# draessld/EDSParser

Measured on AMD Instinct MI355X. Metric: msa2eds_input_MB_per_s, higher is better.
Workload: dtype u8

## Files before the change

### edsparser_amd/csrc/msa_fast_kernels.hpp

```cpp
#pragma once
#include "msa_generic_kernels.hpp"

namespace edsx {

constexpr u64 META_REC = 1ull << 63;
constexpr u64 META_KIND4 = 1ull << 62;
constexpr u64 META_INLINE = 1ull << 61;
constexpr u64 META_KIND8 = 1ull << 60;
constexpr u64 META_RECID = (1ull << 40) - 1;
constexpr u64 CNT_SCATTER = 1ull << 63;
constexpr u64 CNT_SLOT = (1ull << 48) - 1;
constexpr u64 CNT_MIXED = 1ull << 62;
constexpr u32 REC_H_SLOT = 8, REC_H_REP = 16;

__global__ void __launch_bounds__(256) k_seg_meta(FastParams p)
{
    const MsaView& mv = p.mv;
    if (mv.hdr->status) return;
    const u64 nseg = *p.nseg_ptr;
    const u64 p0 = mv.vbit(0) ? 0 : 1;
    const u64 nvs = nseg > p0 ? (nseg - p0 + 1) / 2 : 0;
    if (blockIdx.x == 0 && threadIdx.x == 0) mv.hdr->nvs = nvs;
    auto common = [&](u64 seg, u64 a, u64 b) {
        p.eds_len[seg] = 2 + (b - a);
// ... 11 lines not shown
        if (vi == 0 && p0) common(0, p.seg_start[0], a);
        if (seg + 1 < nseg) common(seg + 1, b, p.seg_start[seg + 2]);
        u64 work_cm = 0, work_wide = 0, work_wide16 = 0;
        bool done = false;
        if (p.Fraw && ((p.Fraw[a >> 6] >> (a & 63)) & 1ull)) {
            const u64 slot = mv.slot(a);
            const u32 info = p.rec_info[slot];
            if (info >> 31) {
                p.eds_len[seg] = (info >> 8) & 0xffu;
                p.seds_len[seg] = (u64)(info & 0xffu) + p.tok_total;
                p.segmeta[seg] = META_REC | META_INLINE | ((info >> 30) & 1u ? META_KIND4 : 0) | slot;
                work_wide = ((info >> 30) & 1u) && (info & 0xffu) <= 8u;
                work_wide16 = ((info >> 30) & 1u) && (info & 0xffu) > 8u;
                done = true;
            }
        }
        if (!done) {
            u64 cm = 0;
            const u64 ncol = b - a;
            if (ncol <= 64) {
                const u64 s0 = mv.slot(a);
                bool pure = true, contig = true;
                for (u64 c = a + 1; c < b; c++) {
                    pure = pure && mv.vbit(c);
                    if (pure) contig = contig && mv.slot(c) == s0 + (c - a);
                }
                if (pure) cm = (ncol << 48) | s0 | (contig ? 0 : CNT_SCATTER);
                else cm = (ncol << 48) | s0 | CNT_MIXED;
            }
            if (!cm) p.slow_list[atomicAdd(p.slow_count, 1ull)] = seg;
            p.segmeta[seg] = 0;
            work_cm = cm;
        }
        const bool heavy = work_cm && ((work_cm & CNT_MIXED) || ((work_cm >> 48) & 0xffu) > 10u);
        p.cnt_meta[vi] = work_cm; p.cnt_flag[vi] = work_cm && !heavy ? 1 : 0; p.heavy_flag[vi] = heavy ? 1 : 0;
        p.wide_flag[vi] = work_wide; p.wide16_flag[vi] = work_wide16;
    }
}

__global__ void __launch_bounds__(256) k_work_scatter(FastParams p, const u64* __restrict__ pos, const u64* __restrict__ hpos,
                                                      const u64* __restrict__ nvs_ptr)
{
    if (p.mv.hdr->status) return;
    const u64 nvs = *nvs_ptr;
    for (u64 vi = blockIdx.x * (u64)blockDim.x + threadIdx.x; vi < nvs; vi += (u64)gridDim.x * blockDim.x) {
        const u64 cm = p.cnt_meta[vi];
        if (cm) {
            const bool heavy = (cm & CNT_MIXED) || ((cm >> 48) & 0xffu) > 10u;
            if (heavy) { const u64 i = hpos[vi]; p.heavy_vi[i] = vi; p.heavy_cm[i] = cm; }
            else { const u64 i = pos[vi]; p.cnt_vi[i] = vi; p.cnt_cm[i] = cm; }
        }
        const u64 wpos = p.wide_flag[vi];
        const u64 wnext = vi + 1 < nvs ? p.wide_flag[vi + 1] : *p.wide_count;
        if (wnext != wpos) p.wide_list[wpos] = vi;
        const u64 xpos = p.wide16_flag[vi];
        const u64 xnext = vi + 1 < nvs ? p.wide16_flag[vi + 1] : *p.wide16_count;
        if (xnext != xpos) p.wide16_list[xpos] = vi;
    }
}

__device__ __forceinline__ uint32_t lut32(const u32* t, uint32_t g4)
{
    const uint32_t sel = g4 & 0x07070707u;
    const uint32_t h3 = (g4 >> 3) & 0x01010101u, m3 = (h3 << 8) - h3;
    const uint32_t h4 = (g4 >> 4) & 0x01010101u, m4 = (h4 << 8) - h4;
    const uint32_t e0 = __builtin_amdgcn_perm(t[1], t[0], sel), e1 = __builtin_amdgcn_perm(t[3], t[2], sel);
    const uint32_t e2 = __builtin_amdgcn_perm(t[5], t[4], sel), e3 = __builtin_amdgcn_perm(t[7], t[6], sel);
    const uint32_t lo = (e1 & m3) | (e0 & ~m3), hi = (e3 & m3) | (e2 & ~m3);
    return (hi & m4) | (lo & ~m4);
}

__device__ __forceinline__ uint32_t lut64(const u32* t, uint32_t g4)
{
    const uint32_t h5 = (g4 >> 5) & 0x01010101u, m5 = (h5 << 8) - h5;
    return (lut32(t + 8, g4) & m5) | (lut32(t, g4) & ~m5);
}

template <int MAXG> __device__ __forceinline__ uint32_t lutN(const u32* t, uint32_t g4)
{
    if constexpr (MAXG <= 8) return __builtin_amdgcn_perm(t[1], t[0], g4);
    else if constexpr (MAXG <= 16) {
// ... 125 lines not shown
    if (ncol == 1) {
        if (fast_group_dna1(col0, rb, vmask, lane, mv.S, G)) return 1;
        G.gid = make_uint4(~0u, ~0u, ~0u, ~0u);
        G.k = 0; G.sumlen = 0; G.key_lo = 0; G.key_hi = 0; G.rep = 0; G.len = 0;
        if (ballot64(any_nul(col0, vmask))) return 0;
        const uint4 col = normalise_col<CHECK_NL>(col0, vmask, saw_nl);
        while (first_remaining(rm, leader, i0)) {
            const u32 c = leader_byte(col, leader, i0);
            uint4 eq = bytes_eq_mask(col, c * 0x01010101u);
            eq.x &= rm.x; eq.y &= rm.y; eq.z &= rm.z; eq.w &= rm.w;
            if (!fast_assign(G, rm, eq, (u64)c, 0ull, c ? 1u : 0u, lane, (u32)leader * 16u + i0)) return 0;
        }
        return 1;
    }

    const u64 slot0 = cmeta & CNT_SLOT;
    const bool scatter = (cmeta & CNT_SCATTER) != 0, mixed = (cmeta & CNT_MIXED) != 0;
    if (mixed && !HEAVY) return 2;
    const u32 loff = lane * 16u < mv.Spad - 16u ? lane * 16u : mv.Spad - 16u;
    const uint8_t* cbase = mv.vc + slot0 * (u64)mv.Spad + loff;
    u32 nA = ncol;
    const uint8_t* cbaseB = cbase;
    const bool two = scatter && mv.lw == 0 && mv.tileW != 0;
    if (two) {
        const u64 bnd = (seg_a / mv.tileW + 1) * mv.tileW;
        nA = (u32)(bnd - seg_a);
        cbaseB = mv.vc + uniform64(mv.word_slot[bnd >> 6]) * (u64)mv.Spad + loff;
    }
    auto col_ptr = [&](u32 c) -> const uint8_t* {
        if (two) return c < nA ? cbase + (u64)c * mv.Spad : cbaseB + (u64)(c - nA) * mv.Spad;
        return scatter ? mv.vc + mv.slot(seg_a + c) * (u64)mv.Spad + loff : cbase + (u64)c * mv.Spad;
    };

    if (!HEAVY && ncol > 10u) return 2;
    if (ncol <= 10u && !mixed) {
        auto load_col = [&](u32 c) -> uint4 { return load16u(col_ptr(c)); };
        const int r = fast_group_dnakeys<1>(load_col, ncol, col0, lane, vmask, G);
        if (r) return r > 0 ? 1 : 0;
        G.gid = make_uint4(~0u, ~0u, ~0u, ~0u);
        G.k = 0; G.sumlen = 0; G.key_lo = 0; G.key_hi = 0; G.rep = 0; G.len = 0;
    }
    if constexpr (HEAVY) {
        if (ncol > 10u && ncol <= 20u && !mixed) {
            auto load_col = [&](u32 c) -> uint4 { return load16u(col_ptr(c)); };
            const int r = fast_group_dnakeys<2>(load_col, ncol, col0, lane, vmask, G);
            if (r) return r > 0 ? 1 : 0;
            G.gid = make_uint4(~0u, ~0u, ~0u, ~0u);
            G.k = 0; G.sumlen = 0; G.key_lo = 0; G.key_hi = 0; G.rep = 0; G.len = 0;
        }
        auto cell_ptr = [&](u32 c) -> const uint8_t* {
            const uint8_t* cp = two ? (c < nA ? cbase + (u64)c * mv.Spad : cbaseB + (u64)(c - nA) * mv.Spad)
                                    : (scatter ? mv.vc + mv.slot(seg_a + c) * (u64)mv.Spad + loff : cbase + (u64)c * mv.Spad);
            return cp - loff;
        };
        u32 cs_lo = 0, cs_hi = 0, cref = 0x100u;
        if (mixed && lane < ncol) {
            if (mv.vbit(seg_a + lane)) { const u64 sl = mv.slot(seg_a + lane); cs_lo = (u32)sl; cs_hi = (u32)(sl >> 32); }
            else cref = mv.ref_byte(seg_a + lane);
        }
        auto load_colx = [&](u32 c) -> uint4 {
            if (mixed) {
                const u32 rb = (u32)__builtin_amdgcn_readlane((int)cref, (int)c);
                if (rb < 0x100u) { const u32 b = rb * 0x01010101u; return make_uint4(b, b, b, b); }
                const u64 sl = ((u64)(u32)__builtin_amdgcn_readlane((int)cs_hi, (int)c) << 32) | (u32)__builtin_amdgcn_readlane((int)cs_lo, (int)c);
                return load16u(mv.vc + sl * (u64)mv.Spad + loff);
            }
            return load16u(col_ptr(c));
        };
        auto cell = [&](u32 c, u32 row) -> u32 {
            if (row == ~0u) return mixed ? (u32)__builtin_amdgcn_readlane((int)cref, (int)c) : 0x100u;
            if (mixed) return cref < 0x100u ? cref : (u32)mv.vc[(((u64)cs_hi << 32) | cs_lo) * (u64)mv.Spad + row];
            return (u32)cell_ptr(c)[row];
        };
        if (mv.S <= 64u && !mixed) {
            const bool act = lane < mv.S;
            u32* const mine32 = reinterpret_cast<u32*>(strs + lane * 64u);
// ... 712 lines not shown
```

### edsparser_amd/csrc/msa_scan_kernels.hpp

```cpp
#pragma once
#include "msa_wave.hpp"
#include "msa_scan_launch.hpp"

namespace edsx {

__global__ void k_find_hdr_end(const uint8_t* __restrict__ f, u64 n, MsaHdr* h)
{
    const u32 lane = threadIdx.x;
    h->first_nl = n;
    h->first_hdr2 = n;
    if (n == 0 || f[0] != '>') {
        if (lane == 0) { h->status |= ST_NOT_FASTA; h->hdr_end = n; }
        return;
    }
    u64 pos = n;
    for (u64 base = 0; base < n; base += 64) {
        u64 i = base + lane;
        u64 b = ballot64(i < n && f[i] == '\n');
        if (b) { pos = base + __builtin_ctzll(b); break; }
    }
    if (lane == 0) h->hdr_end = pos;
}

__global__ void __launch_bounds__(1024) k_find_row0(const uint8_t* __restrict__ f, u64 n, MsaHdr* h)
// ... 147 lines not shown
            u64 nonnl = 0;
            for (u64 i = lane; i < rest; i += 64) nonnl |= (f[p + i] != '\n');
            if (ballot64(nonnl != 0)) bad = ST_LAYOUT;
            break;
        }
        u64 nlpos = n;
        u64 b = ballot64(lane >= 2 && c == '\n');
        if (b) nlpos = q + __builtin_ctzll(b);
        else {
            for (u64 base = q + 64; base < n; base += 64) {
                const u64 i = base + lane;
                b = ballot64(i < n && f[i] == '\n');
                if (b) { nlpos = base + __builtin_ctzll(b); break; }
            }
        }
        if (nlpos >= n) { bad = ST_LAYOUT; break; }
        st = nlpos + 1;
    }
    if (lane == 0) {
        if (s < 2 && !bad) bad = ST_FEW_ROWS;
        h->status |= bad;
        h->S = s; h->L = L; h->lw = wrapped ? lw : 0; h->Draw = Draw;
        h->nwords = (L + 63) / 64;
        h->nwords_raw = (Draw + 63) / 64;
    }
}

__global__ void k_pad_rows(u64* __restrict__ row_start, u64 S, u64 n)
{
    const u64 last = row_start[S - 1];
    for (u64 r = S + blockIdx.x * (u64)blockDim.x + threadIdx.x; r < n; r += (u64)gridDim.x * blockDim.x) row_start[r] = last;
}

constexpr u32 FUSE_MAXW = 10;
#ifndef EDSX_TAIL_WAVES
#define EDSX_TAIL_WAVES 8
#endif
constexpr u32 TAIL_WAVES = EDSX_TAIL_WAVES;
constexpr u32 CLIST = 2048;



template <bool ROWS64>
__device__ __forceinline__ void fused_group_run(const K1Params& p, const uint8_t* colbuf, u32 desc, u64 slot_base, u32 lane,
                                                const uint4& vmask, u32 nl, u32 loff)
{
    const u32 idx0 = desc & 0x7ffu, w = desc >> 11;
    const uint8_t* c0p = colbuf + (size_t)idx0 * p.Spad;
    FastGroups G;
    G.gid = make_uint4(~0u, ~0u, ~0u, ~0u);
    G.k = 0; G.sumlen = 0; G.key_lo = 0; G.key_hi = 0; G.rep = 0; G.len = 0;
    bool ok;
    if constexpr (ROWS64) {
        const bool act = lane < p.S;
        const u64 LET = ((u64)DNA_LET_HI << 32) | DNA_LET_LO;
        u32 klo = 0, khi = 0, len = 0, bad = 0;
        for (u32 c = 0; c < w; c++) {
            const u32 ch = act ? (u32)c0p[(size_t)c * p.Spad + lane] : (u32)'-';
            const u32 cls = ((ch >> 1) ^ (ch >> 2)) & 7u;
            bad |= ((u32)(LET >> (8u * cls)) & 0xffu) != ch ? 1u : 0u;
            if (cls != 5u) { if (len < 10u) klo |= cls << (3u * len); else khi |= cls << (3u * (len - 10u)); len++; }
        }
        ok = !ballot64(act && bad);
        u32 mygid = 0, gk_lo = 0, gk_hi = 0, glen = 0;
        if (ok) {
            u64 todo = ballot64(act);
            while (todo) {
// ... 95 lines not shown
    const u64 q = q0 + (u64)j * 16;
    const bool full_tile = q0 + (u64)cpr * 16 <= p.Draw;
    const int nb = q < p.Draw ? ((p.Draw - q) < 16 ? (int)(p.Draw - q) : 16) : 0;
    const u32 valid = nb == 16 ? 0xffffu : ((1u << nb) - 1u);

    constexpr bool DIRECT_OK = HOLD && LANEROWS;
    const bool direct = DIRECT_OK && full_tile;
    const u64* rs = BIG ? p.row_start : reinterpret_cast<const u64*>(colbuf);
    if (!direct && !BIG) for (u32 r = tid; r < p.S; r += T) reinterpret_cast<u64*>(colbuf)[r] = p.row_start[r];
    if (tid < 256) { D[tid] = 0; CS[tid] = 0; }
    if (tid == 0) { ncand_sh = 0; nst_sh = 0; }
    if (!direct) __syncthreads();

    const uint8_t* f = p.file;
    const u32 Sm1 = p.S - 1;
    auto row_of = [&](u32 it) -> u32 {
        if constexpr (LANEROWS) return sub * 16u + it;
        else return sub + it * RI;
    };
    uint4 ref = make_uint4(0, 0, 0, 0);
    uint4 d[HOLD ? RPT : 1];
    uint4 acc = make_uint4(0, 0, 0, 0);
    if (direct) {
        if constexpr (DIRECT_OK) {
            ref = load16u(f + p.row_start[0] + q);
            const ulonglong2* rp = reinterpret_cast<const ulonglong2*>(p.row_start + sub * 16u);
            ulonglong2 rv[8];
#pragma unroll
            for (int i = 0; i < 8; i++) rv[i] = rp[i];
#pragma unroll
            for (int i = 0; i < 8; i++) { d[2 * i] = load16u(f + rv[i].x + q); d[2 * i + 1] = load16u(f + rv[i].y + q); }
#pragma unroll
            for (int it = 0; it < RPT; it++) {
                acc.x |= d[it].x ^ ref.x; acc.y |= d[it].y ^ ref.y;
                acc.z |= d[it].z ^ ref.z; acc.w |= d[it].w ^ ref.w;
            }
        }
    } else if (full_tile) {
        ref = load16u(f + rs[0] + q);
#pragma unroll
        for (int it = 0; it < RPT; it++) {
            const u32 r = row_of(it);
            d[HOLD ? it : 0] = load16u(f + rs[r < p.S ? r : Sm1] + q);
            if constexpr (!HOLD) {
                acc.x |= d[0].x ^ ref.x; acc.y |= d[0].y ^ ref.y; acc.z |= d[0].z ^ ref.z; acc.w |= d[0].w ^ ref.w;
            }
        }
        if constexpr (HOLD) {
#pragma unroll
            for (int it = 0; it < RPT; it++) {
                acc.x |= d[it].x ^ ref.x; acc.y |= d[it].y ^ ref.y;
                acc.z |= d[it].z ^ ref.z; acc.w |= d[it].w ^ ref.w;
            }
        }
    } else {
        if (nb > 0) ref = load_partial(f + rs[0] + q, nb);
#pragma unroll
        for (int it = 0; it < RPT; it++) {
            const u32 r = row_of(it);
            uint4 v = ref;
            if (r < p.S && nb > 0) v = load_partial(f + rs[r] + q, nb);
            d[HOLD ? it : 0] = v;
            acc.x |= v.x ^ ref.x; acc.y |= v.y ^ ref.y; acc.z |= v.z ^ ref.z; acc.w |= v.w ^ ref.w;
        }
    }
    if constexpr (!HOLD) {
        for (u32 r = sub + RPT * RI; r < p.S; r += RI) {
            if (nb > 0) {
                const uint8_t* src = f + rs[r] + q;
                uint4 v = nb == 16 ? load16u(src) : load_partial(src, nb);
                acc.x |= v.x ^ ref.x; acc.y |= v.y ^ ref.y; acc.z |= v.z ^ ref.z; acc.w |= v.w ^ ref.w;
            }
        }
    }
    u32 diff = chunk_ne16(acc, make_uint4(0, 0, 0, 0));
    diff |= chunk_eq16(ref, 0x2d2d2d2du);
    diff &= valid;
    u32 bad = 0;
    u32 nlmask = 0;
    if (p.lw && nb > 0) {
        u64 m = q % (p.lw + 1);
        for (int i = 0; i < nb; i++) { if (m == p.lw) { nlmask |= 1u << i; m = 0; } else m++; }
    }
    if ((chunk_eq16(ref, 0x0a0a0a0au) & valid) != nlmask) bad = 1;
    if (direct) {
        for (u32 o = cpr; o < 64u; o <<= 1) diff |= (u32)__shfl_xor((int)diff, (int)o, 64);
        __syncthreads();
        if ((tid & 63u) < cpr && diff) atomicOr(&D[j], diff);
    } else if (diff) atomicOr(&D[j], diff);
    __syncthreads();

    const u32 V16 = D[j];
    if (V16 & nlmask) bad = 1;

    const bool fastpre = cpr <= 8u;
    u64 prepk = 0;
    u32 w0 = 0, w1 = 0, w2 = 0, w3 = 0, nv = 0;
    if (fastpre) {
        const uint4 da = *reinterpret_cast<const uint4*>(&D[0]), db = *reinterpret_cast<const uint4*>(&D[4]);
        const u32 dm[8] = {uniform32(da.x), uniform32(da.y), uniform32(da.z), uniform32(da.w),
                           uniform32(db.x), uniform32(db.y), uniform32(db.z), uniform32(db.w)};
#pragma unroll
        for (int c = 0; c < 8; c++) { prepk |= (u64)nv << (8 * c); nv += (u32)__builtin_popcount(dm[c]); }
    } else {
        if (tid < 256) {
            u32 c = tid < cpr ? __builtin_popcount(D[tid]) : 0;
            u32 incl = c;
            for (int o = 1; o < 64; o <<= 1) { u32 a = __shfl_up(incl, o, 64); if ((tid & 63) >= (u32)o) incl += a; }
            if ((tid & 63) == 63) wtot[tid >> 6] = incl;
            pre[tid] = incl - c;
        }
        __syncthreads();
        w0 = wtot[0]; w1 = wtot[1]; w2 = wtot[2]; w3 = wtot[3];
        nv = w0 + w1 + w2 + w3;
    }
    auto pre_of = [&](u32 chunk) -> u32 {
        if (fastpre) return (u32)(prepk >> (8u * (chunk & 7u))) & 0xffu;
        const u32 cw = chunk >> 6;
        return pre[chunk] + (cw > 0 ? w0 : 0u) + (cw > 1 ? w1 : 0u) + (cw > 2 ? w2 : 0u);
    };
    u64 base_r = 0;
    if (tid == 0 && nv) base_r = atomicAdd(&p.hdr->nv, (u64)nv);

    u64 slot_base = 0;
    bool overflow = false;
    {
        const u32 cap = p.cap_cols;
#define EDSX_TCOMP(C, COMP, VISIT) {                                                               \
            uint32_t t4[4][4];                                                                     \
            _Pragma("unroll") for (int k4 = 0; k4 < 4; k4++) {                                    \
                uint32_t a0 = d[4 * k4].COMP, a1 = d[4 * k4 + 1].COMP, a2 = d[4 * k4 + 2].COMP, a3 = d[4 * k4 + 3].COMP; \
                 \
                 \
                asm volatile("" : "+v"(a0), "+v"(a1), "+v"(a2), "+v"(a3));                        \
                const uint32_t t0 = __builtin_amdgcn_perm(a1, a0, 0x05010400u), t1 = __builtin_amdgcn_perm(a1, a0, 0x07030602u); \
                const uint32_t t2 = __builtin_amdgcn_perm(a3, a2, 0x05010400u), t3 = __builtin_amdgcn_perm(a3, a2, 0x07030602u); \
                t4[0][k4] = __builtin_amdgcn_perm(t2, t0, 0x05040100u);                           \
                t4[1][k4] = __builtin_amdgcn_perm(t2, t0, 0x07060302u);                           \
                t4[2][k4] = __builtin_amdgcn_perm(t3, t1, 0x05040100u);                           \
                t4[3][k4] = __builtin_amdgcn_perm(t3, t1, 0x07060302u);                           \
            }                                                                                      \
            VISIT(4 * C, t4[0][0], t4[0][1], t4[0][2], t4[0][3]) VISIT(4 * C + 1, t4[1][0], t4[1][1], t4[1][2], t4[1][3]) \
            VISIT(4 * C + 2, t4[2][0], t4[2][1], t4[2][2], t4[2][3]) VISIT(4 * C + 3, t4[3][0], t4[3][1], t4[3][2], t4[3][3]) }
#define EDSX_TALL(VISIT) EDSX_TCOMP(0, x, VISIT) EDSX_TCOMP(1, y, VISIT) EDSX_TCOMP(2, z, VISIT) EDSX_TCOMP(3, w, VISIT)
        bool fused_tile = false;
        if constexpr (HOLD && LANEROWS) fused_tile = p.fuse && nv && nv <= cap && nv <= CLIST;
        if (fused_tile) { if constexpr (HOLD && LANEROWS) {
            if (V16) {
                uint8_t* dst = colbuf + (size_t)pre_of(j) * p.Spad + (sub * 16u < p.Spad - 16u ? sub * 16u : p.Spad - 16u);
#define EDSX_VISIT(I, A, B, C_, D_) if (V16 & (1u << (I))) { *reinterpret_cast<uint4*>(dst) = make_uint4(A, B, C_, D_); dst += p.Spad; }
                EDSX_TALL(EDSX_VISIT)
#undef EDSX_VISIT
            }
            for (u32 col = tid; col < cpr * 16u; col += T) {
                const u32 ch = col >> 4, b = col & 15u;
                const u32 m = D[ch];
                if ((m >> b) & 1u) {
                    const u64 w = (ch ? (u64)D[ch - 1] : 0xffffull) | ((u64)m << 16) | ((u64)(ch + 1 < cpr ? D[ch + 1] : 0xffffu) << 32) |
                                  ((u64)(ch + 2 < cpr ? D[ch + 2] : 0xffffu) << 48);
                    const u32 pp = 16u + b;
                    const u32 up = (u32)__builtin_ctzll(~(w >> pp));
                    const u32 dn = (u32)__builtin_clzll(~(w << (64u - pp)));
                    const u32 idx = pre_of(ch) + (u32)__builtin_popcount(m & ((1u << b) - 1u));
                    if (up + dn > (ROWS64 ? 20u : FUSE_MAXW) || dn == pp) clist[CLIST - 1u - atomicAdd(&nst_sh, 1u)] = (uint16_t)idx;
                    else if (dn == 0) { clist[atomicAdd(&ncand_sh, 1u)] = (uint16_t)(idx | ((up + dn) << 11)); atomicOr(&CS[ch], 1u << b); }
                }
            }
            if (tid == 0) {
                slot_base_sh = base_r;
                if (base_r + nv > p.vc_cap_cols) atomicOr(&p.hdr->status, (u64)ST_VC_OVERFLOW);
            }
            __syncthreads();
            slot_base = slot_base_sh;
            overflow = slot_base + nv > p.vc_cap_cols;
            if (tid < cpr / 4) {
                u64 wi = q0 / 64 + tid;
                if (wi * 64 < p.Draw) {
                    p.Vraw[wi] = (u64)D[4 * tid] | ((u64)D[4 * tid + 1] << 16) | ((u64)D[4 * tid + 2] << 32) | ((u64)D[4 * tid + 3] << 48);
                    p.word_slot[wi] = slot_base + pre_of(4 * tid);
                    p.Fraw[wi] = (u64)CS[4 * tid] | ((u64)CS[4 * tid + 1] << 16) | ((u64)CS[4 * tid + 2] << 32) | ((u64)CS[4 * tid + 3] << 48);
                }
            }
            if (!overflow) {
                const u32 wv = uniform32(tid >> 6);
                if (wv >= TAIL_WAVES) {
                    if (bad) atomicOr(&p.hdr->status, (u64)(ST_LAYOUT | ST_NEWLINE_IN_DATA));
                    return;
                }
                {
                    const u32 nst = nst_sh, vec = p.Spad / 16u, ln = tid & 63u;
                    for (u32 c = wv; c < nst; c += TAIL_WAVES) {
                        const u32 idx = clist[CLIST - 1u - c];
                        const uint8_t* src = colbuf + (size_t)idx * p.Spad;
                        uint8_t* g = p.vc + (slot_base + idx) * (u64)p.Spad;
                        for (u32 pc = ln; pc < vec; pc += 64u)
                            *reinterpret_cast<uint4*>(g + pc * 16u) = *reinterpret_cast<const uint4*>(src + pc * 16u);
                    }
                }
                const u32 ncand = ncand_sh;
                const u32 lane = tid & 63u, nl = (p.S + 15u) >> 4;
                const uint4 vmask = fast_valid_mask(lane, p.S);
                const u32 loff = lane * 16u < p.Spad - 16u ? lane * 16u : p.Spad - 16u;
                for (u32 ci = wv; ci < ncand; ci += TAIL_WAVES)
                    fused_group_run<ROWS64>(p, colbuf, uniform32((u32)clist[ci]), slot_base, lane, vmask, nl, loff);
            }
        } } else if constexpr (BIG) {
            if (tid == 0) {
                slot_base_sh = base_r;
                if (base_r + nv > p.vc_cap_cols) atomicOr(&p.hdr->status, (u64)ST_VC_OVERFLOW);
            }
            __syncthreads();
            slot_base = slot_base_sh;
            overflow = slot_base + nv > p.vc_cap_cols;
            if (tid < (cpr + 3u) / 4u) {
                const u64 wi = q0 / 64 + tid;
                if (wi * 64 < p.Draw) {
                    p.Vraw[wi] = (u64)D[4 * tid] | ((u64)D[4 * tid + 1] << 16) | ((u64)D[4 * tid + 2] << 32) | ((u64)D[4 * tid + 3] << 48);
                    p.word_slot[wi] = slot_base + pre_of(4 * tid);
                }
            }
            if (nv && !overflow && V16) {
                uint8_t* const dst0 = p.vc + (slot_base + pre_of(j)) * (u64)p.Spad;
                for (u32 r = sub; r < p.S; r += 4 * RI) {
                    uint4 v[4];
#pragma unroll
                    for (int u = 0; u < 4; u++) {
                        const u32 rr = r + (u32)u * RI;
                        v[u] = make_uint4(0, 0, 0, 0);
                        if (rr < p.S) v[u] = nb == 16 ? load16u(f + p.row_start[rr] + q) : load_partial(f + p.row_start[rr] + q, nb);
                    }
#pragma unroll
                    for (int u = 0; u < 4; u++) {
                        const u32 rr = r + (u32)u * RI;
                        if (rr < p.S) {
                            u32 m = V16;
                            uint8_t* dst = dst0 + rr;
                            while (m) {
                                const int i = __builtin_ctz(m);
                                m &= m - 1;
                                const u32 ch = byte_of(v[u], i);
                                if (ch == '\n') bad = 1;
                                *dst = (uint8_t)ch;
                                dst += p.Spad;
// ... 33 lines not shown
                    }
                    EDSX_X(0) EDSX_X(1) EDSX_X(2) EDSX_X(3) EDSX_X(4) EDSX_X(5) EDSX_X(6) EDSX_X(7)
                    EDSX_X(8) EDSX_X(9) EDSX_X(10) EDSX_X(11) EDSX_X(12) EDSX_X(13) EDSX_X(14) EDSX_X(15)
#undef EDSX_X
                } else {
                    for (u32 r = sub; r < p.S; r += 4 * RI) {
                        uint4 v[4];
#pragma unroll
                        for (int u = 0; u < 4; u++) {
                            const u32 rr = r + (u32)u * RI;
                            v[u] = make_uint4(0, 0, 0, 0);
                            if (rr < p.S) v[u] = nb == 16 ? load16u(f + p.row_start[rr] + q) : load_partial(f + p.row_start[rr] + q, nb);
                        }
#pragma unroll
                        for (int u = 0; u < 4; u++) {
                            const u32 rr = r + (u32)u * RI;
                            if (rr < p.S) {
                                u32 m = V16, id = idx;
                                while (m) {
                                    const int i = __builtin_ctz(m);
                                    m &= m - 1;
                                    if (id >= b0 && id < b0 + cap) {
                                        const u32 ch = byte_of(v[u], i);
                                        if (ch == '\n') bad = 1;
                                        colbuf[(size_t)(id - b0) * p.Spad + rr] = (uint8_t)ch;
                                    }
                                    id++;
                                }
                            }
                        }
                    }
                }
            }
            if (b0 == 0 && tid == 0) {
                slot_base_sh = base_r;
                if (base_r + nv > p.vc_cap_cols) atomicOr(&p.hdr->status, (u64)ST_VC_OVERFLOW);
            }
            __syncthreads();
            if (b0 == 0) {
                slot_base = slot_base_sh;
                overflow = slot_base + nv > p.vc_cap_cols;
                if (tid < cpr / 4) {
                    u64 wi = q0 / 64 + tid;
                    if (wi * 64 < p.Draw) {
                        u64 bits = (u64)D[4 * tid] | ((u64)D[4 * tid + 1] << 16) | ((u64)D[4 * tid + 2] << 32) |
                                   ((u64)D[4 * tid + 3] << 48);
                        p.Vraw[wi] = bits;
                        p.word_slot[wi] = slot_base + pre_of(4 * tid);
                        if (p.fuse) p.Fraw[wi] = 0;
                    }
                }
            }
            if (!nv || overflow) break;
            const u32 ncols = (nv - b0) < cap ? (nv - b0) : cap;
            const size_t nbytes = (size_t)ncols * p.Spad;
            uint8_t* g = p.vc + (slot_base + b0) * (u64)p.Spad;
            for (size_t o = (size_t)tid * 16; o < nbytes; o += (size_t)T * 16)
                *reinterpret_cast<uint4*>(g + o) = *reinterpret_cast<const uint4*>(colbuf + o);
            if (b0 + cap < nv) __syncthreads();
        }
    }
    if (bad) atomicOr(&p.hdr->status, (u64)(ST_LAYOUT | ST_NEWLINE_IN_DATA));
}

__global__ void k_vmap(const u64* __restrict__ Vraw, u64* __restrict__ V, u64 L, u64 lw, u64 nwords)
{
    for (u64 w = blockIdx.x * (u64)blockDim.x + threadIdx.x; w < nwords; w += (u64)gridDim.x * blockDim.x) {
        u64 bits = 0;
        for (int i = 0; i < 64; i++) {
            u64 c = w * 64 + i;
// ... 78 lines not shown
```

### edsparser_amd/csrc/msa_wave.hpp

```cpp
#pragma once
#include "msa_device.hpp"

namespace edsx {

enum : u64 {
    ST_NOT_FASTA = 1, ST_LAYOUT = 2, ST_TOO_MANY_ROWS = 4, ST_VC_OVERFLOW = 8,
    ST_NEWLINE_IN_DATA = 16, ST_FEW_ROWS = 32
};

__device__ __forceinline__ u64 uniform64(u64 v)
{
    return ((u64)(u32)__builtin_amdgcn_readfirstlane((int)(u32)(v >> 32)) << 32) |
           (u32)__builtin_amdgcn_readfirstlane((int)(u32)v);
}
__device__ __forceinline__ u32 uniform32(u32 v) { return (u32)__builtin_amdgcn_readfirstlane((int)v); }
__device__ __forceinline__ u64 readlane64(u64 v, int lane)
{
    return ((u64)(u32)__builtin_amdgcn_readlane((int)(u32)(v >> 32), lane) << 32) | (u32)__builtin_amdgcn_readlane((int)(u32)v, lane);
}

__device__ __forceinline__ u64 ld_relaxed(const u64* p)
{
    return __hip_atomic_load(p, __ATOMIC_RELAXED, __HIP_MEMORY_SCOPE_AGENT);
}

__device__ __forceinline__ u32 chunk_ne16(const uint4& a, const uint4& b)
{
    return ne_bytes4(a.x, b.x) | (ne_bytes4(a.y, b.y) << 4) | (ne_bytes4(a.z, b.z) << 8) |
           (ne_bytes4(a.w, b.w) << 12);
}
__device__ __forceinline__ u32 chunk_eq16(const uint4& a, uint32_t cccc)
{
    return eq_byte4(a.x, cccc) | (eq_byte4(a.y, cccc) << 4) | (eq_byte4(a.z, cccc) << 8) |
           (eq_byte4(a.w, cccc) << 12);
}

template <int I> __device__ __forceinline__ u32 byte_at(const uint4& v)
{
    const uint32_t w = I < 4 ? v.x : (I < 8 ? v.y : (I < 12 ? v.z : v.w));
    return (w >> ((I & 3) * 8)) & 0xffu;
}

constexpr int KCAP = 64;
__device__ __forceinline__ uint32_t bytes_ne_mask(uint32_t a, uint32_t b)
{
    uint32_t x = a ^ b;
    uint32_t h = (((x & 0x7f7f7f7fu) + 0x7f7f7f7fu) | x) & 0x80808080u;
    return h | (h - (h >> 7));
}
__device__ __forceinline__ uint4 bytes_eq_mask(const uint4& a, uint32_t cccc)
{
    return make_uint4(~bytes_ne_mask(a.x, cccc), ~bytes_ne_mask(a.y, cccc), ~bytes_ne_mask(a.z, cccc),
                      ~bytes_ne_mask(a.w, cccc));
}
__device__ __forceinline__ bool any4(const uint4& v) { return (v.x | v.y | v.z | v.w) != 0; }
__device__ __forceinline__ bool any_nul(const uint4& c, const uint4& vmask)
{
    const uint4 z = bytes_eq_mask(c, 0u);
    return ((z.x & vmask.x) | (z.y & vmask.y) | (z.z & vmask.z) | (z.w & vmask.w)) != 0;
}
__device__ __forceinline__ u32 first_byte_index(const uint4& m)
{
// ... 160 lines not shown
    u32 vlo = lane < 4u ? rank << (8u * lane) : 0u, vhi = (lane >= 4u && lane < 8u) ? rank << (8u * (lane - 4u)) : 0u;
    vlo |= dpp_move0<0x111, 0xf>(vlo); vhi |= dpp_move0<0x111, 0xf>(vhi);
    vlo |= dpp_move0<0x112, 0xf>(vlo); vhi |= dpp_move0<0x112, 0xf>(vhi);
    vlo |= dpp_move0<0x114, 0xf>(vlo); vhi |= dpp_move0<0x114, 0xf>(vhi);
    const u32 lut_lo = (u32)__builtin_amdgcn_readlane((int)vlo, 7), lut_hi = (u32)__builtin_amdgcn_readlane((int)vhi, 7);
    cls.x |= ~vmask.x; cls.y |= ~vmask.y; cls.z |= ~vmask.z; cls.w |= ~vmask.w;
    G.gid = make_uint4(__builtin_amdgcn_perm(lut_hi, lut_lo, cls.x), __builtin_amdgcn_perm(lut_hi, lut_lo, cls.y),
                       __builtin_amdgcn_perm(lut_hi, lut_lo, cls.z), __builtin_amdgcn_perm(lut_hi, lut_lo, cls.w));
    G.key_lo = 0; G.key_hi = 0; G.rep = 0; G.len = 0;
    for (u32 mm = P; mm; mm &= mm - 1) {
        const u32 c = (u32)__builtin_ctz(mm);
        const u32 r = (u32)__builtin_amdgcn_readlane((int)rank, (int)c), f = (u32)__builtin_amdgcn_readlane((int)firstv, (int)c);
        const u32 letter = c == 5u ? 0u : (u32)((((u64)DNA_LET_HI << 32) | DNA_LET_LO) >> (8u * c)) & 0xffu;
        if (lane == r) { G.key_lo = letter; G.rep = f; G.len = letter ? 1u : 0u; }
    }
    G.k = (u32)__builtin_popcount(P);
    G.sumlen = (u32)__builtin_popcount(P & ~(1u << 5));
    return true;
}

__device__ __forceinline__ bool first_remaining(const uint4& rm, int& leader, u32& i0)
{
    const u64 b = ballot64(any4(rm));
    if (!b) return false;
    leader = __builtin_ctzll(b);
    i0 = (u32)__builtin_amdgcn_readlane((int)first_byte_index(rm), leader);
    return true;
}

template <int NK, class LoadCol>
__device__ __forceinline__ int fast_group_dnakeys(LoadCol load_col, u32 ncol, const uint4& col0, u32 lane, const uint4& vmask,
                                                  FastGroups& G)
{
    u32 key[NK][16];
#pragma unroll
    for (int n = 0; n < NK; n++)
#pragma unroll
        for (int i = 0; i < 16; i++) key[n][i] = 0;
    u32 badacc = 0;
#define EDSX_K(I) key[n][I] |= byte_at<I>(cls) << sh;
#pragma unroll
    for (int n = 0; n < NK; n++) {
        const u32 cbase = 10u * n, cend = ncol < cbase + 10u ? ncol : cbase + 10u;
        for (u32 c0 = cbase; c0 < cend; c0 += 4) {
            uint4 cvs[4];
#pragma unroll
            for (int j = 0; j < 4; j++) {
                cvs[j] = make_uint4(0, 0, 0, 0);
                if (c0 + j < cend) cvs[j] = (c0 + j == 0) ? col0 : load_col(c0 + j);
            }
#pragma unroll
            for (int j = 0; j < 4; j++) {
                if (c0 + j < cend) {
                    const uint4 x = cvs[j];
                    const uint4 cls = dna_classes(x);
                    badacc |= dna_bad(x, cls, vmask);
                    const u32 sh = 3u * (c0 + j - cbase);
                    EDSX_K(0) EDSX_K(1) EDSX_K(2) EDSX_K(3) EDSX_K(4) EDSX_K(5) EDSX_K(6) EDSX_K(7)
                    EDSX_K(8) EDSX_K(9) EDSX_K(10) EDSX_K(11) EDSX_K(12) EDSX_K(13) EDSX_K(14) EDSX_K(15)
                }
            }
        }
    }
#undef EDSX_K
    if (ballot64(badacc != 0)) return 0;
    uint4 rm = vmask;
    int leader;
    u32 i0;
    while (first_remaining(rm, leader, i0)) {
        u32 rk[NK];
#pragma unroll
        for (int n = 0; n < NK; n++) {
            u32 mk = 0;
#pragma unroll
            for (int i = 0; i < 16; i++) mk = (i0 == (u32)i) ? key[n][i] : mk;
            rk[n] = (u32)__builtin_amdgcn_readlane((int)mk, leader);
        }
        uint32_t e[4] = {0, 0, 0, 0};
#pragma unroll
        for (int i = 0; i < 16; i++) {
            bool same = key[0][i] == rk[0];
            if (NK > 1) same = same && key[NK - 1][i] == rk[NK - 1];
            if (same) e[i >> 2] |= 0xffu << ((i & 3) * 8);
        }
        const uint4 eq = make_uint4(e[0] & rm.x, e[1] & rm.y, e[2] & rm.z, e[3] & rm.w);
        u32 cl = 5u;
        if (lane < ncol) cl = ((lane < 10u ? rk[0] : rk[NK - 1]) >> (3u * (lane < 10u ? lane : lane - 10u))) & 7u;
        const u64 nz = ballot64(cl != 5u);
        const u32 len = (u32)__builtin_popcountll(nz), pos = mbcnt(nz);
        u32 klo = 0, khi = 0;
        if (cl != 5u) { if (pos < 10u) klo = cl << (3u * pos); else khi = cl << (3u * (pos - 10u)); }
        klo = wave_or_all(klo);
        if (NK > 1) khi = wave_or_all(khi);
        if (!fast_assign(G, rm, eq, ((u64)khi << 32) | klo, (u64)len << 32, len, lane, (u32)leader * 16u + i0)) return -1;
    }
    return 1;
}


__device__ __forceinline__ u32 pack_gid2(const uint4& gid, const uint4& vmask)
{
    auto p = [](uint32_t x) -> u32 { x &= 0x03030303u; x |= x >> 6; x |= x >> 12; return x & 0xffu; };
    return p(gid.x & vmask.x) | (p(gid.y & vmask.y) << 8) | (p(gid.z & vmask.z) << 16) | (p(gid.w & vmask.w) << 24);
}
__device__ __forceinline__ uint2 pack_gid4(const uint4& gid, const uint4& vmask)
{
    auto p = [](uint32_t x) -> u32 { x &= 0x0f0f0f0fu; x |= x >> 4; return (x & 0xffu) | ((x >> 8) & 0xff00u); };
    return make_uint2(p(gid.x & vmask.x) | (p(gid.y & vmask.y) << 16), p(gid.z & vmask.z) | (p(gid.w & vmask.w) << 16));
}

}
```

### edsparser_amd/csrc/msa_scan.hip

```cpp
#include "msa_scan_kernels.hpp"

namespace edsx {

void launch_find_hdr_end(const uint8_t* f, u64 n, MsaHdr* h, hipStream_t st)
{
    hipLaunchKernelGGL(k_find_hdr_end, dim3(1), dim3(64), 0, st, f, n, h);
}
void launch_find_row0(const uint8_t* f, u64 n, MsaHdr* h, hipStream_t st)
{
    hipLaunchKernelGGL(k_find_row0, dim3(512), dim3(1024), 0, st, f, n, h);
}
void launch_index_spec(const uint8_t* f, u64 n, const MsaHdr* h, u64* hpos, u64* cand, u64 row_cap, hipStream_t st)
{
    hipLaunchKernelGGL(k_index_spec, dim3(512), dim3(256), 0, st, f, n, h, hpos, cand, row_cap);
}
void launch_index_check(const uint8_t* f, u64 n, MsaHdr* h, const u64* hpos, const u64* cand, u64* row_start, u64 row_cap, hipStream_t st)
{
    hipLaunchKernelGGL(k_index_check, dim3(1), dim3(1024), 0, st, f, n, h, hpos, cand, row_start, row_cap);
}
void launch_index_rows(const uint8_t* f, u64 n, MsaHdr* h, u64* row_start, u64 row_cap, hipStream_t st)
{
    hipLaunchKernelGGL(k_index_rows, dim3(1), dim3(64), 0, st, f, n, h, row_start, row_cap);
}
void launch_pad_rows(u64* row_start, u64 S, u64 n, hipStream_t st)
{
    hipLaunchKernelGGL(k_pad_rows, dim3(4), dim3(256), 0, st, row_start, S, n);
}

template <int T, int RPT, bool HOLD, bool LANEROWS, int MINW, bool ROWS64 = false, bool BIG = false>
static void launch_k1(const K1Params& p, size_t lds, hipStream_t st)
{
    auto kern = k_scan_extract<T, RPT, HOLD, LANEROWS, MINW, ROWS64, BIG>;
    EDSX_HIP(hipFuncSetAttribute(reinterpret_cast<const void*>(kern),
                                 hipFuncAttributeMaxDynamicSharedMemorySize, (int)lds));
    hipLaunchKernelGGL(kern, dim3((unsigned)p.ntiles), dim3(T), lds, st, p);
}
void launch_scan_extract(const K1Params& p, int threads, bool hold, bool lane_rows, bool rows64, bool big, size_t lds, hipStream_t st)
{
    if (lane_rows && rows64) launch_k1<512, 16, true, true, 4, true>(p, lds, st);
    else if (lane_rows && threads == 1024) launch_k1<1024, 16, true, true, 4>(p, lds, st);
    else if (lane_rows) launch_k1<512, 16, true, true, 4>(p, lds, st);
    else if (hold) launch_k1<512, 16, true, false, 4>(p, lds, st);
    else if (big) launch_k1<512, 16, false, false, 4, false, true>(p, lds, st);
    else launch_k1<512, 16, false, false, 4>(p, lds, st);
}

void launch_vmap(const u64* Vraw, u64* V, u64 L, u64 lw, u64 nwords, hipStream_t st)
{
    hipLaunchKernelGGL(k_vmap, dim3(1024), dim3(256), 0, st, Vraw, V, L, lw, nwords);
}
void launch_runstart_words(const u64* V, u64* H, u64* cnt, u64 L, u64 nwords, hipStream_t st)
{
    hipLaunchKernelGGL(k_runstart_words, dim3(1024), dim3(256), 0, st, V, H, cnt, L, nwords);
}
void launch_write_positions(const u64* H, const u64* wbase, u64* pos, u64 nwords, const u64* total, u64 L, hipStream_t st)
{
    hipLaunchKernelGGL(k_write_positions, dim3(1024), dim3(256), 0, st, H, wbase, pos, nwords, total, L);
}
void launch_seg_flags(const u64* run_start, const u64* V, const u64* R_ptr, u64 l, u64* flag, hipStream_t st)
{
    hipLaunchKernelGGL(k_seg_flags, dim3(1024), dim3(256), 0, st, run_start, V, R_ptr, l, flag);
}
void launch_write_segs(const u64* run_start, const u64* flag, const u64* sidx, const u64* R_ptr, const u64* nseg_ptr, u64* seg_start,
                       u64* Hseg, u64 L, hipStream_t st)
{
    hipLaunchKernelGGL(k_write_segs, dim3(1024), dim3(256), 0, st, run_start, flag, sidx, R_ptr, nseg_ptr, seg_start, Hseg, L);
}
void launch_popc_words(const u64* H, u64* cnt, u64 nwords, hipStream_t st)
{
    hipLaunchKernelGGL(k_popc_words, dim3(1024), dim3(256), 0, st, H, cnt, nwords);
}

}
```

Measured before the change: 2.769 million.

## Pack DNA column keys in base-6 bytes to fit twelve columns per key dword

Replaces the 3-bit-per-column key packing in fast_group_dnakeys with a base-6 encoding. Each byte holds three columns as d0+6d1+36d2, built with byte-permute table lookups and adds, and the bytes are then transposed into per-row dwords. This raises the single-dword column limit from 10 to 12, so more segments take the light and fused-scan paths instead of the heavy ones, and FUSE_MAXW goes up to match. Decoding now needs a multiply-based digit extraction per lane, and the extra khi reduction runs when ncol exceeds 10.

Measured after the change: 2.782 million (median of 6 runs). About the same (+0.5%).

```diff
diff --git a/edsparser_amd/csrc/msa_fast_kernels.hpp b/edsparser_amd/csrc/msa_fast_kernels.hpp
--- a/edsparser_amd/csrc/msa_fast_kernels.hpp
+++ b/edsparser_amd/csrc/msa_fast_kernels.hpp
@@ -67,7 +67,7 @@
             p.segmeta[seg] = 0;
             work_cm = cm;
         }
-        const bool heavy = work_cm && ((work_cm & CNT_MIXED) || ((work_cm >> 48) & 0xffu) > 10u);
+        const bool heavy = work_cm && ((work_cm & CNT_MIXED) || ((work_cm >> 48) & 0xffu) > LIGHT_MAXW);
         p.cnt_meta[vi] = work_cm; p.cnt_flag[vi] = work_cm && !heavy ? 1 : 0; p.heavy_flag[vi] = heavy ? 1 : 0;
         p.wide_flag[vi] = work_wide; p.wide16_flag[vi] = work_wide16;
     }
@@ -81,7 +81,7 @@
     for (u64 vi = blockIdx.x * (u64)blockDim.x + threadIdx.x; vi < nvs; vi += (u64)gridDim.x * blockDim.x) {
         const u64 cm = p.cnt_meta[vi];
         if (cm) {
-            const bool heavy = (cm & CNT_MIXED) || ((cm >> 48) & 0xffu) > 10u;
+            const bool heavy = (cm & CNT_MIXED) || ((cm >> 48) & 0xffu) > LIGHT_MAXW;
             if (heavy) { const u64 i = hpos[vi]; p.heavy_vi[i] = vi; p.heavy_cm[i] = cm; }
             else { const u64 i = pos[vi]; p.cnt_vi[i] = vi; p.cnt_cm[i] = cm; }
         }
@@ -273,8 +273,8 @@
         return scatter ? mv.vc + mv.slot(seg_a + c) * (u64)mv.Spad + loff : cbase + (u64)c * mv.Spad;
     };
 
-    if (!HEAVY && ncol > 10u) return 2;
-    if (ncol <= 10u && !mixed) {
+    if (!HEAVY && ncol > LIGHT_MAXW) return 2;
+    if (ncol <= LIGHT_MAXW && !mixed) {
         auto load_col = [&](u32 c) -> uint4 { return load16u(col_ptr(c)); };
         const int r = fast_group_dnakeys<1>(load_col, ncol, col0, lane, vmask, G);
         if (r) return r > 0 ? 1 : 0;
@@ -282,7 +282,7 @@
         G.k = 0; G.sumlen = 0; G.key_lo = 0; G.key_hi = 0; G.rep = 0; G.len = 0;
     }
     if constexpr (HEAVY) {
-        if (ncol > 10u && ncol <= 20u && !mixed) {
+        if (ncol > LIGHT_MAXW && ncol <= KEYS2_MAXW && !mixed) {
             auto load_col = [&](u32 c) -> uint4 { return load16u(col_ptr(c)); };
             const int r = fast_group_dnakeys<2>(load_col, ncol, col0, lane, vmask, G);
             if (r) return r > 0 ? 1 : 0;
diff --git a/edsparser_amd/csrc/msa_key6.hpp b/edsparser_amd/csrc/msa_key6.hpp
--- /dev/null
+++ b/edsparser_amd/csrc/msa_key6.hpp
@@ -0,0 +1,37 @@
+#pragma once
+#include <cstdint>
+
+#if defined(__HIPCC__)
+#define EDSX_HD __host__ __device__ __forceinline__
+#else
+#define EDSX_HD inline
+#endif
+
+namespace edsx {
+
+constexpr uint32_t KEY6_COLS = 12;
+constexpr uint32_t LIGHT_MAXW = KEY6_COLS;
+constexpr uint32_t KEYS2_MAXW = 20;
+static_assert(KEYS2_MAXW <= 2 * KEY6_COLS, "two key dwords per row");
+constexpr uint32_t KEY6_GAP = 5;
+
+EDSX_HD uint32_t key6_digit_of_class(uint32_t cls) { return (0x30540210u >> (4u * cls)) & 0xfu; }
+EDSX_HD uint32_t key6_class_of_digit(uint32_t d) { return (0x547210u >> (4u * d)) & 0xfu; }
+
+constexpr uint32_t key6_table(uint32_t scale, bool hi)
+{
+    uint32_t t = 0;
+    for (uint32_t i = 0; i < 4; i++) t |= (((0x30540210u >> (4u * (i + (hi ? 4u : 0u)))) & 0xfu) * scale) << (8u * i);
+    return t;
+}
+
+EDSX_HD uint32_t key6_encode3(uint32_t d0, uint32_t d1, uint32_t d2) { return d0 + 6u * d1 + 36u * d2; }
+
+EDSX_HD uint32_t key6_mul(uint32_t p) { return p == 0 ? 65536u : (p == 1 ? 10923u : 1821u); }
+EDSX_HD uint32_t key6_digit(uint32_t b, uint32_t mul)
+{
+    const uint32_t q = (b * mul) >> 16;
+    return q - 6u * ((q * 10923u) >> 16);
+}
+
+}
diff --git a/edsparser_amd/csrc/msa_scan_kernels.hpp b/edsparser_amd/csrc/msa_scan_kernels.hpp
--- a/edsparser_amd/csrc/msa_scan_kernels.hpp
+++ b/edsparser_amd/csrc/msa_scan_kernels.hpp
@@ -203,7 +203,8 @@
     for (u64 r = S + blockIdx.x * (u64)blockDim.x + threadIdx.x; r < n; r += (u64)gridDim.x * blockDim.x) row_start[r] = last;
 }
 
-constexpr u32 FUSE_MAXW = 10;
+constexpr u32 FUSE_MAXW = 12;
+static_assert(FUSE_MAXW <= KEY6_COLS, "the scan groups with one key dword per row");
 #ifndef EDSX_TAIL_WAVES
 #define EDSX_TAIL_WAVES 8
 #endif
diff --git a/edsparser_amd/csrc/msa_wave.hpp b/edsparser_amd/csrc/msa_wave.hpp
--- a/edsparser_amd/csrc/msa_wave.hpp
+++ b/edsparser_amd/csrc/msa_wave.hpp
@@ -1,5 +1,6 @@
 #pragma once
 #include "msa_device.hpp"
+#include "msa_key6.hpp"
 
 namespace edsx {
 
@@ -254,38 +255,53 @@
 __device__ __forceinline__ int fast_group_dnakeys(LoadCol load_col, u32 ncol, const uint4& col0, u32 lane, const uint4& vmask,
                                                   FastGroups& G)
 {
+    constexpr u32 D1_LO = key6_table(1, false), D1_HI = key6_table(1, true), D6_LO = key6_table(6, false), D6_HI = key6_table(6, true);
+    constexpr u32 D36_LO = key6_table(36, false), D36_HI = key6_table(36, true);
     u32 key[NK][16];
-#pragma unroll
-    for (int n = 0; n < NK; n++)
-#pragma unroll
-        for (int i = 0; i < 16; i++) key[n][i] = 0;
     u32 badacc = 0;
-#define EDSX_K(I) key[n][I] |= byte_at<I>(cls) << sh;
 #pragma unroll
     for (int n = 0; n < NK; n++) {
-        const u32 cbase = 10u * n, cend = ncol < cbase + 10u ? ncol : cbase + 10u;
-        for (u32 c0 = cbase; c0 < cend; c0 += 4) {
-            uint4 cvs[4];
-#pragma unroll
-            for (int j = 0; j < 4; j++) {
-                cvs[j] = make_uint4(0, 0, 0, 0);
-                if (c0 + j < cend) cvs[j] = (c0 + j == 0) ? col0 : load_col(c0 + j);
-            }
-#pragma unroll
-            for (int j = 0; j < 4; j++) {
-                if (c0 + j < cend) {
-                    const uint4 x = cvs[j];
-                    const uint4 cls = dna_classes(x);
-                    badacc |= dna_bad(x, cls, vmask);
-                    const u32 sh = 3u * (c0 + j - cbase);
-                    EDSX_K(0) EDSX_K(1) EDSX_K(2) EDSX_K(3) EDSX_K(4) EDSX_K(5) EDSX_K(6) EDSX_K(7)
-                    EDSX_K(8) EDSX_K(9) EDSX_K(10) EDSX_K(11) EDSX_K(12) EDSX_K(13) EDSX_K(14) EDSX_K(15)
+        const u32 cbase = KEY6_COLS * n, cend = ncol < cbase + KEY6_COLS ? ncol : cbase + KEY6_COLS;
+        uint4 tr[4];
+#pragma unroll
+        for (int h = 0; h < 2; h++) {
+            tr[2 * h] = make_uint4(0, 0, 0, 0); tr[2 * h + 1] = make_uint4(0, 0, 0, 0);
+            const u32 c0 = cbase + 6u * h;
+            if (c0 < cend) {
+                uint4 cvs[6];
+#pragma unroll
+                for (int j = 0; j < 6; j++) {
+                    cvs[j] = make_uint4(0, 0, 0, 0);
+                    if (c0 + j < cend) cvs[j] = (c0 + j == 0) ? col0 : load_col(c0 + j);
+                }
+#pragma unroll
+                for (int j = 0; j < 6; j++) {
+                    if (c0 + j < cend) {
+                        const uint4 x = cvs[j];
+                        const uint4 cls = dna_classes(x);
+                        badacc |= dna_bad(x, cls, vmask);
+                        const u32 TH = j % 3 == 0 ? D1_HI : (j % 3 == 1 ? D6_HI : D36_HI);
+                        const u32 TL = j % 3 == 0 ? D1_LO : (j % 3 == 1 ? D6_LO : D36_LO);
+                        uint4& t = tr[2 * h + j / 3];
+                        t.x += __builtin_amdgcn_perm(TH, TL, cls.x); t.y += __builtin_amdgcn_perm(TH, TL, cls.y);
+                        t.z += __builtin_amdgcn_perm(TH, TL, cls.z); t.w += __builtin_amdgcn_perm(TH, TL, cls.w);
+                    }
                 }
             }
         }
-    }
-#undef EDSX_K
+#define EDSX_KT(Q, COMP) {                                                                                          \
+            const uint32_t t0 = __builtin_amdgcn_perm(tr[1].COMP, tr[0].COMP, 0x05010400u), t1 = __builtin_amdgcn_perm(tr[1].COMP, tr[0].COMP, 0x07030602u); \
+            const uint32_t t2 = __builtin_amdgcn_perm(tr[3].COMP, tr[2].COMP, 0x05010400u), t3 = __builtin_amdgcn_perm(tr[3].COMP, tr[2].COMP, 0x07030602u); \
+            key[n][4 * Q] = __builtin_amdgcn_perm(t2, t0, 0x05040100u); key[n][4 * Q + 1] = __builtin_amdgcn_perm(t2, t0, 0x07060302u);   \
+            key[n][4 * Q + 2] = __builtin_amdgcn_perm(t3, t1, 0x05040100u); key[n][4 * Q + 3] = __builtin_amdgcn_perm(t3, t1, 0x07060302u); }
+        EDSX_KT(0, x) EDSX_KT(1, y) EDSX_KT(2, z) EDSX_KT(3, w)
+#undef EDSX_KT
+    }
     if (ballot64(badacc != 0)) return 0;
+    const u32 lcol = lane < KEY6_COLS ? lane : lane - KEY6_COLS;
+    const u32 lsh = 8u * (lcol / 3u), lmul = key6_mul(lcol % 3u);
+    const bool lhi = NK > 1 && lane >= KEY6_COLS;
+    const bool need_hi = NK > 1 || ncol > 10u;
     uint4 rm = vmask;
     int leader;
     u32 i0;
@@ -306,14 +322,14 @@
             if (same) e[i >> 2] |= 0xffu << ((i & 3) * 8);
         }
         const uint4 eq = make_uint4(e[0] & rm.x, e[1] & rm.y, e[2] & rm.z, e[3] & rm.w);
-        u32 cl = 5u;
-        if (lane < ncol) cl = ((lane < 10u ? rk[0] : rk[NK - 1]) >> (3u * (lane < 10u ? lane : lane - 10u))) & 7u;
-        const u64 nz = ballot64(cl != 5u);
+        u32 cl = KEY6_GAP;
+        if (lane < ncol) cl = key6_class_of_digit(key6_digit(((lhi ? rk[NK - 1] : rk[0]) >> lsh) & 0xffu, lmul));
+        const u64 nz = ballot64(cl != KEY6_GAP);
         const u32 len = (u32)__builtin_popcountll(nz), pos = mbcnt(nz);
         u32 klo = 0, khi = 0;
-        if (cl != 5u) { if (pos < 10u) klo = cl << (3u * pos); else khi = cl << (3u * (pos - 10u)); }
+        if (cl != KEY6_GAP) { if (pos < 10u) klo = cl << (3u * pos); else khi = cl << (3u * (pos - 10u)); }
         klo = wave_or_all(klo);
-        if (NK > 1) khi = wave_or_all(khi);
+        if (need_hi) khi = wave_or_all(khi);
         if (!fast_assign(G, rm, eq, ((u64)khi << 32) | klo, (u64)len << 32, len, lane, (u32)leader * 16u + i0)) return -1;
     }
     return 1;
```

## Fuse xor-or accumulation into bitop3 and force VGPR atomic addressing

Applied to the files above, without the earlier changes.

Replaces the paired XOR and OR in the row-compare accumulation with a single three-input bitop3 instruction per 32-bit word. The atomic slot reservation and the publication of the slot base now use empty asm barriers that keep the address and result in vector registers, likely to avoid scalar/vector transfers or waitcnt stalls. It also removes the dispatch to the hold/non-lane-rows kernel variant, so that configuration now falls through to the big or default variant. The intent is fewer ALU instructions in a memory-bound scan, at the risk of changing which kernel variant runs when hold is set.

New measurement: 2.758 million before, 2.826 million after, median of 6. 1.02x the previous value.

```diff
diff --git a/edsparser_amd/csrc/msa_scan.hip b/edsparser_amd/csrc/msa_scan.hip
--- a/edsparser_amd/csrc/msa_scan.hip
+++ b/edsparser_amd/csrc/msa_scan.hip
@@ -40,7 +40,6 @@
     if (lane_rows && rows64) launch_k1<512, 16, true, true, 4, true>(p, lds, st);
     else if (lane_rows && threads == 1024) launch_k1<1024, 16, true, true, 4>(p, lds, st);
     else if (lane_rows) launch_k1<512, 16, true, true, 4>(p, lds, st);
-    else if (hold) launch_k1<512, 16, true, false, 4>(p, lds, st);
     else if (big) launch_k1<512, 16, false, false, 4, false, true>(p, lds, st);
     else launch_k1<512, 16, false, false, 4>(p, lds, st);
 }
diff --git a/edsparser_amd/csrc/msa_scan_kernels.hpp b/edsparser_amd/csrc/msa_scan_kernels.hpp
--- a/edsparser_amd/csrc/msa_scan_kernels.hpp
+++ b/edsparser_amd/csrc/msa_scan_kernels.hpp
@@ -365,8 +365,7 @@
             for (int i = 0; i < 8; i++) { d[2 * i] = load16u(f + rv[i].x + q); d[2 * i + 1] = load16u(f + rv[i].y + q); }
 #pragma unroll
             for (int it = 0; it < RPT; it++) {
-                acc.x |= d[it].x ^ ref.x; acc.y |= d[it].y ^ ref.y;
-                acc.z |= d[it].z ^ ref.z; acc.w |= d[it].w ^ ref.w;
+                acc_or_xor(acc, d[it], ref);
             }
         }
     } else if (full_tile) {
@@ -376,14 +375,13 @@
             const u32 r = row_of(it);
             d[HOLD ? it : 0] = load16u(f + rs[r < p.S ? r : Sm1] + q);
             if constexpr (!HOLD) {
-                acc.x |= d[0].x ^ ref.x; acc.y |= d[0].y ^ ref.y; acc.z |= d[0].z ^ ref.z; acc.w |= d[0].w ^ ref.w;
+                acc_or_xor(acc, d[0], ref);
             }
         }
         if constexpr (HOLD) {
 #pragma unroll
             for (int it = 0; it < RPT; it++) {
-                acc.x |= d[it].x ^ ref.x; acc.y |= d[it].y ^ ref.y;
-                acc.z |= d[it].z ^ ref.z; acc.w |= d[it].w ^ ref.w;
+                acc_or_xor(acc, d[it], ref);
             }
         }
     } else {
@@ -394,7 +392,7 @@
             uint4 v = ref;
             if (r < p.S && nb > 0) v = load_partial(f + rs[r] + q, nb);
             d[HOLD ? it : 0] = v;
-            acc.x |= v.x ^ ref.x; acc.y |= v.y ^ ref.y; acc.z |= v.z ^ ref.z; acc.w |= v.w ^ ref.w;
+            acc_or_xor(acc, v, ref);
         }
     }
     if constexpr (!HOLD) {
@@ -402,7 +400,7 @@
             if (nb > 0) {
                 const uint8_t* src = f + rs[r] + q;
                 uint4 v = nb == 16 ? load16u(src) : load_partial(src, nb);
-                acc.x |= v.x ^ ref.x; acc.y |= v.y ^ ref.y; acc.z |= v.z ^ ref.z; acc.w |= v.w ^ ref.w;
+                acc_or_xor(acc, v, ref);
             }
         }
     }
@@ -453,7 +451,18 @@
         return pre[chunk] + (cw > 0 ? w0 : 0u) + (cw > 1 ? w1 : 0u) + (cw > 2 ? w2 : 0u);
     };
     u64 base_r = 0;
-    if (tid == 0 && nv) base_r = atomicAdd(&p.hdr->nv, (u64)nv);
+    if (tid == 0 && nv) {
+        u32 zero = 0;
+        asm volatile("" : "+v"(zero));
+        base_r = atomicAdd(&p.hdr->nv + zero, (u64)nv);
+    }
+    auto publish_slot = [&]() {
+        u32 lo = (u32)base_r, hi = (u32)(base_r >> 32);
+        asm volatile("" : "+v"(lo), "+v"(hi));
+        const u64 b = ((u64)hi << 32) | lo;
+        slot_base_sh = b;
+        if (b + nv > p.vc_cap_cols) atomicOr(&p.hdr->status, (u64)ST_VC_OVERFLOW);
+    };
 
     u64 slot_base = 0;
     bool overflow = false;
@@ -499,10 +508,7 @@
                     else if (dn == 0) { clist[atomicAdd(&ncand_sh, 1u)] = (uint16_t)(idx | ((up + dn) << 11)); atomicOr(&CS[ch], 1u << b); }
                 }
             }
-            if (tid == 0) {
-                slot_base_sh = base_r;
-                if (base_r + nv > p.vc_cap_cols) atomicOr(&p.hdr->status, (u64)ST_VC_OVERFLOW);
-            }
+            if (tid == 0) publish_slot();
             __syncthreads();
             slot_base = slot_base_sh;
             overflow = slot_base + nv > p.vc_cap_cols;
@@ -538,10 +544,7 @@
                     fused_group_run<ROWS64>(p, colbuf, uniform32((u32)clist[ci]), slot_base, lane, vmask, nl, loff);
             }
         } } else if constexpr (BIG) {
-            if (tid == 0) {
-                slot_base_sh = base_r;
-                if (base_r + nv > p.vc_cap_cols) atomicOr(&p.hdr->status, (u64)ST_VC_OVERFLOW);
-            }
+            if (tid == 0) publish_slot();
             __syncthreads();
             slot_base = slot_base_sh;
             overflow = slot_base + nv > p.vc_cap_cols;
@@ -641,10 +644,7 @@
                     }
                 }
             }
-            if (b0 == 0 && tid == 0) {
-                slot_base_sh = base_r;
-                if (base_r + nv > p.vc_cap_cols) atomicOr(&p.hdr->status, (u64)ST_VC_OVERFLOW);
-            }
+            if (b0 == 0 && tid == 0) publish_slot();
             __syncthreads();
             if (b0 == 0) {
                 slot_base = slot_base_sh;
diff --git a/edsparser_amd/csrc/msa_wave.hpp b/edsparser_amd/csrc/msa_wave.hpp
--- a/edsparser_amd/csrc/msa_wave.hpp
+++ b/edsparser_amd/csrc/msa_wave.hpp
@@ -28,6 +28,13 @@
 {
     return ne_bytes4(a.x, b.x) | (ne_bytes4(a.y, b.y) << 4) | (ne_bytes4(a.z, b.z) << 8) |
            (ne_bytes4(a.w, b.w) << 12);
+}
+__device__ __forceinline__ void acc_or_xor(uint4& acc, const uint4& row, const uint4& ref)
+{
+    constexpr uint32_t TA = 0xF0u, TB = 0xCCu, TC = 0xAAu, TT = TA | (TB ^ TC);
+    static_assert(TT == 0xF6u, "a | (b ^ c)");
+    acc.x = __builtin_amdgcn_bitop3_b32(acc.x, row.x, ref.x, TT); acc.y = __builtin_amdgcn_bitop3_b32(acc.y, row.y, ref.y, TT);
+    acc.z = __builtin_amdgcn_bitop3_b32(acc.z, row.z, ref.z, TT); acc.w = __builtin_amdgcn_bitop3_b32(acc.w, row.w, ref.w, TT);
 }
 __device__ __forceinline__ u32 chunk_eq16(const uint4& a, uint32_t cccc)
 {
```
